# carlson-lab/redcliff-s-hypothesizing-dynamic-causal-graphs

Hardware: AMD Instinct MI355X
Metric: cMLP-factor fwd+bwd windows/sec/GPU; grid-search fits/hour on 8 GPUs (higher is better)
Workload: dtype f32; 1 GPU; REDCLIFF-S cMLP w/ state smoothing, D4IC-shaped (p=10, gen_lag=4, K=4, h=100, DGCNN F=20/2 layers/30 hidden), combined-phase batch_update, B=128; global_batch=128, parallelism=replicas1 (one independent fit per GPU, no collective), ranks=1, world_size=1

## Files before the change

redcliff-s-hypothesizing-dynamic-causal-graphs_amd/csrc/rc_common.h:

```cpp
#pragma once
#include <hip/hip_runtime.h>
#include <hip/hip_ext.h>
#include <stdint.h>
#include "redcliff_hip.h"

#define RC_BLOCK 256
#define RC_TRACE_FLOATS 32768
#define RC_LDS_LIMIT_FLOATS 16384
#define RC_LDS_MAX_FLOATS 40960
#define RC_MAX_ACTIVE 256

struct EmbOff {
  int64_t A, gcW, bnw, bnb, fc1W, fc1b, fc2W, fc2b, total;
};
struct FacOff {
  int64_t W0, b0, W1, b1, total;
};
struct WsOff {
  int64_t T;
  int64_t R;
  int64_t f1;
  int64_t w;
  int64_t a;
  int64_t y;
// ... 208 lines not shown
  put(o.w1, K * eh);
  put(o.g, K * p * d.F);
  put(o.g0, K * p);
  put(o.E, p * p * Ls);
  put(o.E0, p * p);
  put(o.dE, K * p * p * Ls);
  put(o.draw, B * K);
  o.total = x;
  if (next) *next = nr;
  return o;
}
struct CEmbCtx {
  int eh;
  float* ws; int64_t wss;
  CEmbPOff po;
  CEmbWsOff wo;
};

#define LP_FACTOR 0
#define LP_FWL1 1
#define LP_COS 2
#define LP_SMOOTH 3
#define ACC_FORECAST 0
#define ACC_FACTOR 1
#define ACC_COS 2
#define ACC_FWL1 3
#define ACC_SMOOTH 4
#define ACC_ADJ 5
#define ACC_COMBO 6
#define ACC_BATCHES 7

enum {
  RC_MG_F, RC_MG_P, RC_MG_PF, RC_MG_NF, RC_MG_K, RC_MG_M1, RC_MG_H, RC_MG_L, RC_MG_B, RC_MG_NPF, RC_MG_PH,
  RC_MG_CS, RC_MG_CSF, RC_MG_NCSF, RC_MG_CSH, RC_MG_LS, RC_MG_LSF, RC_MG_NLSF, RC_MG_LSH, RC_MG_NCH, RC_MG_ENBW,
  RC_MG_ZS, RC_MG_Q, RC_MG_NU, RC_MG_N
};

struct StepCtx {
  RedcliffDims d;
  int B, Lmax, Ls, flags, nbn;
  int Bg;
  int tA, tB;
  const float* X; int64_t xr; int64_t row0;
  const float* lab; int64_t labr;
  const double* bns; int64_t bnsr;
  float *emb, *embM, *embV; int64_t es;
  float *fac, *facM, *facV; int64_t fs;
  float *rm, *rv;
  const RedcliffReplicaHyper* hyp;
  float* ws; int64_t wss;
  double* acc;
  int* conf;
  float *gE, *gF;
  int dsN, dgN, dwN;
  int64_t dsCC, dsS, dsI;
  int fslots;
  int defer;
  EmbOff eo;
  FacOff fo;
  WsOff wo;
  int nrep, rident;
  int wait_dbg;
  uint8_t rmap[RC_MAX_ACTIVE];
  unsigned mg[RC_MG_N];
  int ewpb, enbwm, enbw;
  int fzs;
  const float* cE;
  float* cdE;
  int64_t cwss;
  const float* adt;
  int adi;
};

__host__ __device__ inline int rc_rep(const StepCtx& c, int i) { return c.rident ? i : (int)c.rmap[i]; }
inline int rc_rep_host(const StepCtx& c, int i) { return rc_rep(c, i); }

#define RC_KID_EMB_FWD 0
#define RC_KID_FAC_FWD 1
#define RC_KID_FAC_BWD 2
#define RC_KID_EMB_BWD 3
#define RC_KID_EMB_FINAL 4
#define RC_KID_FAC_MIX 5
#define RC_KID_EMB_WAIT 7
#ifdef RC_TRACE
#define RC_WG_MARK(wsbase, total, kid, end)                                                        \
  do {                                                                                            \
    if (threadIdx.x == 0 && blockIdx.y == 0 && blockIdx.z == 0 && blockIdx.x < 1024)               \
      reinterpret_cast<unsigned long long*>((wsbase) + (total) - RC_TRACE_FLOATS)[(kid) * 2048 + 2 * blockIdx.x + (end)] = \
          wall_clock64();                                                                         \
  } while (0)
#define RC_PHASE(wsbase, total, bx, i)                                                            \
  do {                                                                                            \
    if (threadIdx.x == 0 && (bx) == 0 && blockIdx.y == 0 && blockIdx.z == 0)                       \
      reinterpret_cast<unsigned long long*>((wsbase) + (total) - RC_TRACE_FLOATS)[6 * 2048 + (i)] = wall_clock64(); \
  } while (0)
#else
#define RC_WG_MARK(wsbase, total, kid, end) \
  do {                                      \
  } while (0)
#define RC_PHASE(wsbase, total, bx, i) \
  do {                                 \
  } while (0)
#endif


__device__ inline void rc_store_sc1(float* p, float v) {
  __hip_atomic_store(reinterpret_cast<unsigned*>(p), __float_as_uint(v), __ATOMIC_RELAXED, __HIP_MEMORY_SCOPE_AGENT);
}
__device__ inline float rc_load_sc1(const float* p) {
  return __uint_as_float(
      __hip_atomic_load(reinterpret_cast<unsigned*>(const_cast<float*>(p)), __ATOMIC_RELAXED, __HIP_MEMORY_SCOPE_AGENT));
}
__device__ inline void rc_store_payload(float* p, float v, bool sc1) {
  if (sc1)
    rc_store_sc1(p, v);
  else
    *p = v;
}

#define RC_PUB_DWP 0u
#define RC_PUB_ALL 16u
__device__ inline void rc_publish(unsigned* cnt, unsigned shift) {
  asm volatile("s_waitcnt vmcnt(0)" ::: "memory");
  __syncthreads();
  if (threadIdx.x == 0) __hip_atomic_fetch_add(cnt, 1u << shift, __ATOMIC_RELAXED, __HIP_MEMORY_SCOPE_AGENT);
}

#define RC_WAIT_POLLS (1u << 24)
#define RC_WAIT_POLLS_DBG (1u << 12)

__device__ inline void rc_wait_count(const unsigned* cnt, unsigned shift, unsigned target, unsigned* status, unsigned polls) {
  if (threadIdx.x == 0) {
    unsigned spins = 0;
    while (((__hip_atomic_load(const_cast<unsigned*>(cnt), __ATOMIC_RELAXED, __HIP_MEMORY_SCOPE_AGENT) >> shift) & 0xffffu) < target) {
      if (++spins >= polls) {
        __hip_atomic_fetch_add(status, 1u, __ATOMIC_RELAXED, __HIP_MEMORY_SCOPE_AGENT);
        break;
      }
      __builtin_amdgcn_s_sleep(2);
    }
  }
  __builtin_amdgcn_fence(__ATOMIC_ACQUIRE, "wavefront");
  __syncthreads();
}

__device__ inline unsigned* rc_fac_lead_cnt(const StepCtx& c, float* ws) {
  return reinterpret_cast<unsigned*>(ws + c.wo.ecnt) + c.d.p * ((c.d.H + EMB_HC - 1) / EMB_HC);
}
__device__ inline void rc_wait_leads(const StepCtx& c, float* ws, const unsigned* cnt, unsigned shift, unsigned target) {
  rc_wait_count(cnt, shift, target + (c.wait_dbg ? 1u : 0u), reinterpret_cast<unsigned*>(ws + c.wo.errw),
                c.wait_dbg ? RC_WAIT_POLLS_DBG : RC_WAIT_POLLS);
}

__device__ inline float rc_wave_sum(float v) {
#pragma unroll
  for (int o = 32; o > 0; o >>= 1) v += __shfl_xor(v, o, 64);
  return v;
}

__host__ __device__ inline int64_t rc_y_idx(const RedcliffDims& d, int slot, int kj, int b) {
  return ((int64_t)slot * d.K * d.p + kj) * d.Bmax + b;
}

__device__ inline void rc_xcd_order(int nx, int nz, int& x, int& z) {
  if ((nz & 7) != 0) return;
  const int L = x + nx * z, slot = L >> 3, q = slot / nx;
  x = slot - q * nx;
  z = (L & 7) + 8 * q;
}

__host__ __device__ inline unsigned long long rc_magic40(long long d) {
  return d > 1 ? ((1ull << 40) + (unsigned long long)d - 1) / (unsigned long long)d : 0ull;
}

struct RcDiv {
  unsigned long long m;
  int d;
  __device__ inline explicit RcDiv(int dd) : m(rc_magic40(dd)), d(dd) {}
  __device__ inline int div(int n) const {
    return d == 1 ? n : (int)(((unsigned long long)(unsigned)n * m) >> 40);
  }
  __device__ inline int mod(int n) const { return n - div(n) * d; }
};

__host__ __device__ inline unsigned rc_magic32(long long d) {
  return d > 1 ? (unsigned)(((1ull << 32) + (unsigned long long)d - 1) / (unsigned long long)d) : 0u;
}
struct RcDiv32 {
  unsigned m;
  int d;
  __device__ inline RcDiv32(int dd, unsigned mm) : m(mm), d(dd) {}
  __device__ inline explicit RcDiv32(int dd) : m(rc_magic32(dd)), d(dd) {}
  __device__ inline int div(int n) const { return d == 1 ? n : (int)__umulhi((unsigned)n, m); }
  __device__ inline int mod(int n) const { return n - div(n) * d; }
};

template <int U, int NT = RC_BLOCK, class Ld, class St>
__device__ inline void rc_stage(int N, Ld ld, St st) {
  for (int base = threadIdx.x; base < N; base += U * NT) {
    float v[U];
#pragma unroll
    for (int u = 0; u < U; ++u) {
      const int e = base + u * NT;
      v[u] = e < N ? ld(e) : 0.f;
    }
#pragma unroll
    for (int u = 0; u < U; ++u) {
      const int e = base + u * NT;
      if (e < N) st(e, v[u]);
    }
  }
}

template <int U, int NT, class Ld, class St>
struct RcSeg {
  int N;
  Ld ld;
  St st;
  float v[U];
  __device__ inline bool active(int r) const { return r * U * NT < N; }
  __device__ inline void load(int r) {
#pragma unroll
    for (int u = 0; u < U; ++u) {
      const int e = r * U * NT + u * NT + (int)threadIdx.x;
      v[u] = e < N ? ld(e) : 0.f;
    }
  }
  __device__ inline void store(int r) {
#pragma unroll
    for (int u = 0; u < U; ++u) {
      const int e = r * U * NT + u * NT + (int)threadIdx.x;
      if (e < N) st(e, v[u]);
    }
  }
};
template <int U, int NT = RC_BLOCK, class Ld, class St>
__device__ inline RcSeg<U, NT, Ld, St> rc_seg(int N, Ld ld, St st) {
  return RcSeg<U, NT, Ld, St>{N, ld, st, {}};
}
template <class... S>
__device__ inline void rc_stage_all(S&&... s) {
  for (int r = 0; (s.active(r) || ...); ++r) {
    (s.load(r), ...);
    (s.store(r), ...);
  }
}

template <int U, int NT, class Ld, class St>
struct RcSegC {
  int N;
  Ld ld;
  St st;
  float v[U];
  __device__ inline bool active(int r) const { return r * U * NT < N; }
  __device__ inline void load(int r) {
#pragma unroll
    for (int u = 0; u < U; ++u) {
      const int e0 = (r * U + u) * NT;
      if (e0 < N) v[u] = ld(min(e0 + (int)threadIdx.x, N - 1));
    }
  }
  __device__ inline void store(int r) {
#pragma unroll
    for (int u = 0; u < U; ++u) {
      const int e0 = (r * U + u) * NT, e = e0 + (int)threadIdx.x;
      if (e0 < N && e < N) st(e, v[u]);
    }
  }
};
template <int U, int NT = RC_BLOCK, class Ld, class St>
__device__ inline RcSegC<U, NT, Ld, St> rc_segc(int N, Ld ld, St st) {
  return RcSegC<U, NT, Ld, St>{N, ld, st};
}

struct RcWin {
  const float* base;
  int Tp, p, L, Q;
  unsigned mQ, mp, mL;
};
__device__ __forceinline__ RcWin rc_win(const StepCtx& c, const float* X, int b0) {
  const RedcliffDims& d = c.d;
  return RcWin{X + ((c.row0 + b0) * d.T + (c.Lmax - d.L)) * d.p, d.T * d.p, d.p, d.L, d.p * d.L,
               c.mg[RC_MG_Q], c.mg[RC_MG_P], c.mg[RC_MG_L]};
}
template <int U, int TWL, int NT>
struct RcWinSeg {
  RcWin w;
  int N, nb, q0, stride, padto;
  bool slab;
  float* tile;
  float v[U];
  __device__ __forceinline__ bool active(int r) const { return r * U * NT < N; }
  __device__ __forceinline__ void load(int r) {
    if (slab) {
      const RcDiv32 dQ(w.Q, w.mQ);
#pragma unroll
      for (int u = 0; u < U; ++u) {
        const int e0 = (r * U + u) * NT;
        if (e0 < N) {
          const int e = min(e0 + (int)threadIdx.x, N - 1), b = dQ.div(e);
          v[u] = w.base[(unsigned)(e + b * (w.Tp - w.Q))];
        }
      }
    } else {
      const RcDiv32 dL(w.L, w.mL);
#pragma unroll
      for (int u = 0; u < U; ++u) {
        const int e0 = (r * U + u) * NT;
        if (e0 < N) {
          const int e = min(e0 + (int)threadIdx.x, N - 1), b = e >> TWL, q = q0 + (e & ((1 << TWL) - 1));
          const bool in = q < w.Q;
          const int qc = in ? q : 0, ch = dL.div(qc), t = qc - ch * w.L;
          const float x = w.base[(unsigned)(b * w.Tp + t * w.p + ch)];
          v[u] = in ? x : 0.f;
        }
      }
    }
  }
  __device__ __forceinline__ void store(int r) {
    if (slab) {
      const RcDiv32 dQ(w.Q, w.mQ), dp(w.p, w.mp);
#pragma unroll
      for (int u = 0; u < U; ++u) {
        const int e0 = (r * U + u) * NT, e = e0 + (int)threadIdx.x;
        if (e0 < N && e < N) {
          const int b = dQ.div(e), s = e - b * w.Q, t = dp.div(s), ch = s - t * w.p;
          tile[b * stride + ch * w.L + t] = v[u];
        }
      }
      const int pw = padto - w.Q;
      if (r == 0 && pw > 0 && N > 0) {
        const int sh = pw <= 16 ? 4 : (pw <= 32 ? 5 : 6), col = (int)threadIdx.x & ((1 << sh) - 1);
        if (col < pw)
          for (int b = (int)threadIdx.x >> sh; b < nb; b += NT >> sh) tile[b * stride + w.Q + col] = 0.f;
      }
    } else {
#pragma unroll
      for (int u = 0; u < U; ++u) {
        const int e0 = (r * U + u) * NT, e = e0 + (int)threadIdx.x;
        if (e0 < N && e < N) tile[(e >> TWL) * stride + (e & ((1 << TWL) - 1))] = v[u];
      }
    }
  }
};
template <int U, int TWL, int NT = RC_BLOCK>
__device__ __forceinline__ RcWinSeg<U, TWL, NT> rc_win_seg(const RcWin w, bool slab, int nb, int q0, float* tile, int stride, int padto) {
  RcWinSeg<U, TWL, NT> s;
  s.w = w;
  s.N = slab ? nb * w.Q : nb << TWL;
  s.nb = nb; s.q0 = q0; s.stride = stride; s.padto = padto;
  s.slab = slab;
  s.tile = tile;
  return s;
}

__device__ inline void rc_critical_priority() { __builtin_amdgcn_s_setprio(2); }

typedef float f32x16 __attribute__((ext_vector_type(16)));
typedef float f32x4 __attribute__((ext_vector_type(4)));
__device__ inline int mf_row(int reg, int lane) { return (reg & 3) + 8 * (reg >> 2) + 4 * (lane >> 5); }

template <int NB, bool CLAMP, class LA, class LB, class PA, class PB>
__device__ __forceinline__ f32x4 rc_mfma_chain16(f32x4 acc, int n, int lg, LA la, LB lb, PA pa, PB pb) {
  for (int k0 = 0; k0 < n; k0 += 4 * NB) {
    float av[NB], bv[NB];
#pragma unroll
    for (int s = 0; s < NB; ++s) {
      const int k = k0 + 4 * s + lg, kc = CLAMP ? min(k, n - 1) : k;
      av[s] = la(kc);
      bv[s] = lb(kc);
    }
    __builtin_amdgcn_sched_barrier(0);
#pragma unroll
    for (int s = 0; s < NB; ++s) {
      const int k = k0 + 4 * s + lg;
      if (k0 + 4 * s >= n) break;
      acc = __builtin_amdgcn_mfma_f32_16x16x4f32(pa(k) ? av[s] : 0.f, pb(k) ? bv[s] : 0.f, acc, 0, 0, 0);
    }
  }
  return acc;
}
template <int NB, bool CLAMP, class LA, class LB>
__device__ __forceinline__ f32x4 rc_mfma_chain16(f32x4 acc, int n, int lg, LA la, LB lb) {
  auto in = [n](int k) { return k < n; };
  return rc_mfma_chain16<NB, CLAMP>(acc, n, lg, la, lb, in, in);
}

__device__ inline float rc_block_sum(float v, float* red) {
  v = rc_wave_sum(v);
  const int lane = threadIdx.x & 63, wv = threadIdx.x >> 6;
  __syncthreads();
  if (lane == 0) red[wv] = v;
  __syncthreads();
  float s = 0.f;
  for (int i = 0; i < (int)(blockDim.x >> 6); ++i) s += red[i];
  __syncthreads();
  return s;
// ... 181 lines not shown
```

redcliff-s-hypothesizing-dynamic-causal-graphs_amd/csrc/rc_forward.hip:

```cpp
#include <cstdlib>
#include <cstring>
#include <type_traits>

#include "rc_common.h"

namespace {

#define FK_BT 128
#define FQ_MAX 96
#define RC_EMB_TEAM_NT 512
#ifndef FF_KB
#define FF_KB 4
#endif

__device__ inline int fq_tile(const RedcliffDims& d) { return d.p * d.L <= FQ_MAX ? d.p * d.L : 32; }

template <int NBT, int NT>
__device__ __attribute__((always_inline)) void emb_fwd_body(const StepCtx& c, int bx, int SB, int w_lds, int cs, int zs, float* sm) {
  constexpr bool TEAM = NT == RC_EMB_TEAM_NT;
  constexpr int UD = NT / RC_BLOCK;
  const RedcliffDims& d = c.d;
  const int r = rc_rep(c, blockIdx.y);
  const int b0 = bx * SB;
  const int nb = min(SB, c.B - b0);
  if (nb <= 0) return;
  const int Zs = cs == (int)c.mg[RC_MG_CS] ? c.fzs : (d.p + cs - 1) / cs;
  const int zlo = zs < 0 ? 0 : zs, zhi = zs < 0 ? Zs : zs + 1;
  const int ch0 = zlo * cs, ch1 = min(d.p, zhi * cs);
  RC_WG_MARK(c.ws, c.wo.total, RC_KID_EMB_FWD, 0);
  RC_PHASE(c.ws, c.wo.total, bx, 0);
  const int p = d.p, F = d.F, H = d.H, n = d.n, M1 = d.M1, K = d.K;
  const int pF = p * F, pH = p * H, nFH = n * F * H;
  const RcDiv32 dF(F, c.mg[RC_MG_F]), dp(p, c.mg[RC_MG_P]), dpF(pF, c.mg[RC_MG_PF]), dH(H, c.mg[RC_MG_H]);
  const float* E = c.emb + r * c.es;
  float* ws = c.ws + r * c.wss;
  const float* X = c.X + r * c.xr;
  const int tid = threadIdx.x;

  float* xs = sm;
  float* Sl = xs + SB * pF;
  float* Wl = Sl + n * p * p;
  float* Tl = Wl + (w_lds ? nFH : 0);
  float* Rl = Tl + SB * n * pF;
  float* f1l = Rl + SB * pH;
  float* fc2s = f1l + SB * M1;
  float* fb1 = fc2s + K * M1;
  float* fb2 = fb1 + M1;
  float* alpha = fb2 + K;
  float* beta = alpha + F;
  float* partl = beta + F;

  if (blockIdx.x == 0) {
    unsigned* cnt = reinterpret_cast<unsigned*>(ws + c.wo.ecnt);
    for (int e = tid; e < p * rc_nchunk(d); e += NT) cnt[e] = 0u;
  }
  RC_PHASE(c.ws, c.wo.total, bx, 1);
  const bool train = c.flags & RC_BN_TRAIN;
  double st_mean = 0.0, st_var = 0.0;
  float bw = 0.f, bb = 0.f;
  if (tid < F) {
    if (train) {
      st_mean = c.bns[r * c.bnsr + tid];
      st_var = c.bns[r * c.bnsr + F + tid];
    } else {
      st_mean = c.rm[r * F + tid];
      st_var = c.rv[r * F + tid];
    }
    bw = E[c.eo.bnw + tid];
    bb = E[c.eo.bnb + tid];
  }
  const float* S = ws + c.wo.S;
  const float* gw = E + c.eo.gcW;
  rc_stage_all(
      rc_seg<2 / UD, NT>(n * p * p, [&](int e) { return S[e]; }, [&](int e, float v) { Sl[e] = v; }),
      rc_seg<20 / UD, NT>(w_lds ? nFH : 0, [&](int e) { return gw[e]; }, [&](int e, float v) { Wl[e] = v; }),
      rc_seg<4 / UD, NT>(nb * pF, [&](int e) {
        const int s = dpF.div(e), rem = e - s * pF;
        return X[(c.row0 + b0 + s) * d.T * p + (int64_t)(c.Lmax - F) * p + rem];
      }, [&](int e, float v) {
        const int s = dpF.div(e), rem = e - s * pF, f = dp.div(rem), ch = rem - f * p;
        xs[s * pF + ch * F + f] = v;
      }),
      rc_seg<4 / UD, NT>(K * M1, [&](int e) { return E[c.eo.fc2W + e]; }, [&](int e, float v) { fc2s[e] = v; }),
      rc_seg<1, NT>(M1 + K, [&](int e) { return e < M1 ? E[c.eo.fc1b + e] : E[c.eo.fc2b + e - M1]; },
                [&](int e, float v) { fb1[e] = v; }));
  RC_PHASE(c.ws, c.wo.total, bx, 2);
  if (tid < F) {
    const float mean = (float)st_mean;
    const float inv = train ? (float)(1.0 / sqrt(st_var + c.hyp[r].bn_eps))
                            : 1.0f / sqrtf((float)st_var + (float)c.hyp[r].bn_eps);
    const float a = inv * bw;
    alpha[tid] = a;
    beta[tid] = bb - mean * a;
  }
  __syncthreads();
  for (int e = tid; e < nb * pF; e += NT) {
    const int f = dF.mod(e);
    xs[e] = xs[e] * alpha[f] + beta[f];
  }
  __syncthreads();
  RC_PHASE(c.ws, c.wo.total, bx, 3);
  const int cF = (ch1 - ch0) * F, cH = (ch1 - ch0) * H;
  const int cw = ch1 - ch0;
  const int mb = cw == (int)c.mg[RC_MG_CS] ? RC_MG_CSF : (cw == (int)c.mg[RC_MG_LS] ? RC_MG_LSF : -1);
  const RcDiv32 dcF = mb >= 0 ? RcDiv32(cF, c.mg[mb]) : (cw == p ? RcDiv32(cF, c.mg[RC_MG_PF]) : RcDiv32(cF));
  const RcDiv32 dncF = mb >= 0 ? RcDiv32(n * cF, c.mg[mb + 1]) : (cw == p ? RcDiv32(n * cF, c.mg[RC_MG_NPF]) : RcDiv32(n * cF));
  const RcDiv32 dcH = mb >= 0 ? RcDiv32(cH, c.mg[mb + 2]) : (cw == p ? RcDiv32(cH, c.mg[RC_MG_PH]) : RcDiv32(cH));
  for (int e = tid; e < nb * n * cF; e += NT) {
    const int s = dncF.div(e), rs = e - s * n * cF, i = dcF.div(rs), qs = rs - i * cF;
    const int q = ch0 * F + qs, rem = i * pF + q, ch = dF.div(q), f = q - ch * F;
    float v;
    if (i == 0) {
      v = xs[s * pF + q];
    } else {
      v = 0.f;
      const float* Srow = Sl + (i * p + ch) * p;
      const float* xc = xs + s * pF + f;
      for (int cc = 0; cc < p; ++cc) v += Srow[cc] * xc[cc * F];
    }
    Tl[s * n * pF + rem] = v;
    ws[c.wo.T + (int64_t)(b0 + s) * n * pF + rem] = v;
  }
  __syncthreads();
  RC_PHASE(c.ws, c.wo.total, bx, 4);
  const float* W1 = E + c.eo.fc1W;
  const int lane = tid & 63, wv = __builtin_amdgcn_readfirstlane(tid >> 6) & 3;
  const int team = TEAM ? __builtin_amdgcn_readfirstlane(tid >> 8) : 0;
  const int fz0 = TEAM ? min(team, Zs) : zlo, fz1 = TEAM ? min(team + 1, Zs) : zhi;
  const int RW = (M1 + 3) / 4, m0 = wv * RW;
  auto qend = [&](int z) { return min(p, (z + 1) * cs) * H; };
  int qb = qend(fz0);
  auto ldw = [&](float (&w)[16], int qn) {
    const int qc = qn < qb ? qn : qb - 1;
#pragma unroll
    for (int j = 0; j < 16; ++j) w[j] = (j < RW && m0 + j < M1) ? W1[(int64_t)(m0 + j) * pH + qc] : 0.f;
  };
  float wb0[16], wb1[16], wb2[16];
  if (fz0 < fz1) {
    ldw(wb0, fz0 * cs * H + lane);
    ldw(wb1, fz0 * cs * H + lane + 64);
  }
  RC_PHASE(c.ws, c.wo.total, bx, 5);
  const float* Wsrc = w_lds ? Wl : gw;
  for (int e = tid; e < nb * cH; e += NT) {
    const int s = dcH.div(e), rem = ch0 * H + (e - s * cH), ch = dH.div(rem), hh = rem - ch * H;
    float a4[4] = {0.f, 0.f, 0.f, 0.f};
    for (int i = 0; i < n; ++i) {
      const float* trow = Tl + (s * n + i) * pF + ch * F;
      const float* wc = Wsrc + i * F * H + hh;
      int f = 0;
      for (; f + 3 < F; f += 4) {
#pragma unroll
        for (int u = 0; u < 4; ++u) a4[u] += trow[f + u] * wc[(f + u) * H];
      }
      for (; f < F; ++f) a4[0] += trow[f] * wc[f * H];
    }
    const float v = fmaxf((a4[0] + a4[1]) + (a4[2] + a4[3]), 0.f);
    Rl[s * pH + rem] = v;
    ws[c.wo.R + (int64_t)(b0 + s) * pH + rem] = v;
  }
  __syncthreads();
  RC_PHASE(c.ws, c.wo.total, bx, 6);
  const int jrow = (lane >> 2) & 15, mrow = m0 + jrow;
  const bool wrow = (lane & 3) == 0 && jrow < RW && mrow < M1;
  auto fc1 = [&](auto nbc) {
    constexpr int NB = decltype(nbc)::value;
    float tot[NB];
    for (int z = fz0; z < fz1; ++z) {
      const int qa = z * cs * H;
      qb = qend(z);
      if (z > fz0) {
        ldw(wb0, qa + lane);
        ldw(wb1, qa + lane + 64);
      }
      float acc[16][NB];
#pragma unroll
      for (int j = 0; j < 16; ++j)
#pragma unroll
        for (int s = 0; s < NB; ++s) acc[j][s] = 0.f;
      auto mul = [&](const float (&w)[16], int q) {
        if (q < qb) {
          float rv[NB];
#pragma unroll
          for (int s = 0; s < NB; ++s) rv[s] = s < nb ? Rl[s * pH + q] : 0.f;
#pragma unroll
          for (int j = 0; j < 16; ++j)
#pragma unroll
            for (int s = 0; s < NB; ++s) acc[j][s] += w[j] * rv[s];
        }
      };
      for (int q0 = qa; q0 < qb; q0 += 192) {
        const int q = q0 + lane;
        ldw(wb2, q + 128);
        mul(wb0, q);
        if (q0 + 64 >= qb) break;
        ldw(wb0, q + 192);
        mul(wb1, q + 64);
        if (q0 + 128 >= qb) break;
        ldw(wb1, q + 256);
        mul(wb2, q + 128);
      }
#pragma unroll
      for (int s = 0; s < NB; ++s) {
        if (s >= nb) break;
        float v[16];
#pragma unroll
        for (int j = 0; j < 16; ++j) v[j] = acc[j][s];
#pragma unroll
        for (int half = 8; half >= 1; half >>= 1) {
          const int off = half * 4;
          const bool hi = lane & off;
#pragma unroll
          for (int i = 0; i < half; ++i) {
            const float send = hi ? v[i] : v[i + half];
            const float keep = hi ? v[i + half] : v[i];
            v[i] = keep + __shfl_xor(send, off, 64);
          }
        }
        float t = v[0];
        t += __shfl_xor(t, 2, 64);
        t += __shfl_xor(t, 1, 64);
        tot[s] = z == fz0 ? t : tot[s] + t;
      }
    }
    if (TEAM) {
      if (wrow && fz0 < fz1) partl[team * M1 + mrow] = tot[0];
    } else if (zs < 0) {
#pragma unroll
      for (int s = 0; s < NB; ++s) {
        if (s >= nb) break;
        if (wrow) {
          const float val = tot[s] + fb1[mrow];
          f1l[s * M1 + mrow] = val;
          ws[c.wo.f1 + (int64_t)(b0 + s) * M1 + mrow] = val;
        }
      }
    } else if (wrow) {
      rc_store_sc1(ws + c.wo.f1p + ((int64_t)zs * d.Bmax + b0) * M1 + mrow, tot[0]);
    }
  };
  fc1(std::integral_constant<int, NBT>{});
  if (TEAM) {
    __syncthreads();
    RC_PHASE(c.ws, c.wo.total, bx, 12);
    if (tid < M1) {
      const float val = Zs > 1 ? (partl[tid] + partl[M1 + tid]) + fb1[tid] : partl[tid] + fb1[tid];
      f1l[tid] = val;
      ws[c.wo.f1 + (int64_t)b0 * M1 + tid] = val;
    }
  } else if (zs >= 0) {
    __shared__ unsigned last;
    unsigned* cnt = reinterpret_cast<unsigned*>(ws + c.wo.ecnt) + p * rc_nchunk(d) + 1 + b0;
    asm volatile("s_waitcnt vmcnt(0)" ::: "memory");
    __syncthreads();
    if (tid == 0) last = __hip_atomic_fetch_add(cnt, 1u, __ATOMIC_RELAXED, __HIP_MEMORY_SCOPE_AGENT) == (unsigned)(Zs - 1);
    __syncthreads();
    if (!last) return;
    if (tid == 0) __hip_atomic_store(cnt, 0u, __ATOMIC_RELAXED, __HIP_MEMORY_SCOPE_AGENT);
    __builtin_amdgcn_fence(__ATOMIC_ACQUIRE, "wavefront");
    if (tid < M1) {
      const float* part = ws + c.wo.f1p + (int64_t)b0 * M1 + tid;
      float sum = 0.f;
      for (int z0 = 0; z0 < Zs; z0 += 8) {
        float v[8];
#pragma unroll
        for (int u = 0; u < 8; ++u) v[u] = z0 + u < Zs ? rc_load_sc1(part + (int64_t)(z0 + u) * d.Bmax * M1) : 0.f;
#pragma unroll
        for (int u = 0; u < 8; ++u)
          if (z0 + u < Zs) sum = z0 + u == 0 ? v[0] : sum + v[u];
      }
      const float val = sum + fb1[tid];
      f1l[tid] = val;
      ws[c.wo.f1 + (int64_t)b0 * M1 + tid] = val;
    }
  }
  __syncthreads();
  RC_PHASE(c.ws, c.wo.total, bx, 7);
  for (int e = tid; e < nb * K; e += NT) {
    const int s = e / K, k = e - s * K;
    const float* w2 = fc2s + k * M1;
    float a = 0.f;
    for (int m = 0; m < M1; ++m) a += w2[m] * fmaxf(f1l[s * M1 + m], 0.f);
    ws[c.wo.w + (int64_t)(b0 + s) * K + k] = a + fb2[k];
  }
  RC_PHASE(c.ws, c.wo.total, bx, 8);
  RC_WG_MARK(c.ws, c.wo.total, RC_KID_EMB_FWD, 1);
}

size_t emb_fwd_floats(const RedcliffDims& d, int SB, int w_lds, bool team = false) {
  const size_t pF = (size_t)d.p * d.F, pH = (size_t)d.p * d.H;
  return SB * pF + (size_t)d.n * d.p * d.p + (w_lds ? (size_t)d.n * d.F * d.H : 0) + SB * d.n * pF + SB * pH +
         (size_t)SB * d.M1 + (size_t)d.K * d.M1 + d.M1 + d.K + 2 * d.F + (team ? 2 * d.M1 : 0);
}

template <int NT, bool MF>
__device__ __attribute__((always_inline)) void fac_fwd_body(const StepCtx& c, int bx, float* sm) {
  constexpr int UD = NT / RC_BLOCK, NI = FK_BT * FAC_UC / NT;
  const RedcliffDims& d = c.d;
  RC_WG_MARK(c.ws, c.wo.total, RC_KID_FAC_FWD, 0);
  const int nU = rc_nuchunk(d);
  const int r = rc_rep(c, blockIdx.y), kj = RcDiv32(nU, c.mg[RC_MG_NU]).div(bx), uc = bx - kj * nU;
  const int p = d.p, h = d.h, K = d.K;
  const int Q = p * d.L, QT = fq_tile(d), QP = QT + 1;
  const bool slab = Q <= FQ_MAX;
  const int u0 = uc * FAC_UC;
  const float* P = c.fac + r * c.fs;
  const float* W0 = P + c.fo.W0 + (int64_t)kj * h * Q;
  const float* b0 = P + c.fo.b0 + (int64_t)kj * h;
  const float* W1 = P + c.fo.W1 + (int64_t)kj * h;
  const float b1 = uc == 0 ? P[c.fo.b1 + kj] : 0.f;
  float* ws = c.ws + r * c.wss;
  const float* X = c.X + r * c.xr;
  const int tid = threadIdx.x, tb = tid >> 4, tu = tid & 15;
  const int u = u0 + tu;
  const RcDiv32 dQ(Q, c.mg[RC_MG_Q]);
  float* Xs = sm;
  float* Ws = Xs + FK_BT * QP;
  const int nrow = min(FAC_UC, h - u0);
  const float* W0c = W0 + u0 * Q;
  const float bu = u < h ? b0[u] : 0.f, w1 = u < h ? W1[u] : 0.f;
  const bool mf = MF && slab;
  const int lane = tid & 63, fwv = __builtin_amdgcn_readfirstlane(tid >> 6), l15 = lane & 15, lg = lane >> 4;
  float bu4[4], w14[4];
#pragma unroll
  for (int reg = 0; reg < 4; ++reg) {
    const int uu = u0 + 4 * lg + reg;
    bu4[reg] = mf && uu < h ? b0[uu] : 0.f;
    w14[reg] = mf && uu < h ? W1[uu] : 0.f;
  }

  for (int bc = 0; bc < c.B; bc += FK_BT) {
    float acc[NI];
#pragma unroll
    for (int i = 0; i < NI; ++i) acc[i] = 0.f;
    for (int q0 = 0; q0 < Q; q0 += QT) {
      if (q0 > 0 || bc > 0) __syncthreads();
      rc_stage_all(
          rc_win_seg<24 / UD, 5, NT>(rc_win(c, X, bc), slab, min(FK_BT, c.B - bc), q0, Xs, QP, Q),
          rc_segc<4 / UD, NT>(slab ? nrow * Q : 0, [&](int e) { return W0c[(unsigned)e]; }, [&](int e, float v) {
            const int uu = dQ.div(e);
            Ws[uu * QP + e - uu * Q] = v;
          }),
          rc_segc<2 / UD, NT>(slab ? 0 : FAC_UC * 32, [&](int e) {
            const int uu = e >> 5, q = q0 + (e & 31);
            const bool in = uu < nrow && q < Q;
            const float w = W0c[(unsigned)(in ? uu * Q + q : 0)];
            return in ? w : 0.f;
          }, [&](int e, float v) { Ws[(e >> 5) * QP + (e & 31)] = v; }));
      if (slab)
        for (int e = nrow * QP + tid; e < FAC_UC * QP; e += NT) Ws[e] = 0.f;
      __syncthreads();
      if (bc == 0 && q0 == 0) RC_PHASE(c.ws, c.wo.total, bx, 64);
      if (bc == 0)
        for (int qq = tid; qq < QT && q0 + qq < Q; qq += NT) {
          float sq = 0.f;
          for (int uu = 0; uu < FAC_UC; ++uu) {
            const float w = Ws[uu * QP + qq];
            sq += w * w;
          }
          ws[c.wo.gq + ((int64_t)uc * K * p + kj) * Q + q0 + qq] = sq;
        }
      if (bc == 0 && q0 == 0) RC_PHASE(c.ws, c.wo.total, bx, 65);
      if (mf) break;
      const int qn = min(QT, Q - q0);
#pragma unroll 8
      for (int qq = 0; qq < qn; ++qq) {
        const float wv = Ws[tu * QP + qq];
#pragma unroll
        for (int i = 0; i < NI; ++i) acc[i] = fmaf(Xs[(tb + (NT / 16) * i) * QP + qq], wv, acc[i]);
      }
    }
    if (bc == 0 && tb == 0 && u < h) ws[c.wo.w1 + (int64_t)kj * h + u] = w1;
    if (mf) {
      const float* wr = Ws + l15 * QP;
      for (int bt = fwv; bt < (min(FK_BT, c.B - bc) + 15) / 16; bt += NT / 64) {
        const float* xr = Xs + (16 * bt + l15) * QP;
        const f32x4 z = rc_mfma_chain16<FF_KB, true>(
            f32x4{0.f, 0.f, 0.f, 0.f}, Q, lg, [&](int kc) { return wr[kc]; }, [&](int kc) { return xr[kc]; });
        if (bc == 0 && bt == 0) RC_PHASE(c.ws, c.wo.total, bx, 66);
        const int b = bc + 16 * bt + l15;
        float ys[4];
#pragma unroll
        for (int reg = 0; reg < 4; ++reg) {
          const int uu = u0 + 4 * lg + reg;
          ys[reg] = 0.f;
          if (uu < h) {
            const float a = fmaxf(z[reg] + bu4[reg], 0.f);
            if (b < c.B && !rc_fac_recompute(d)) ws[c.wo.a + ((int64_t)kj * d.Bmax + b) * h + uu] = a;
            ys[reg] = w14[reg] * a;
          }
        }
#pragma unroll
        for (int reg = 0; reg < 4; ++reg) ys[reg] += __shfl_xor(ys[reg], 32, 64);
#pragma unroll
        for (int reg = 0; reg < 4; ++reg) ys[reg] += __shfl_xor(ys[reg], 16, 64);
        const float y = (ys[0] + ys[2]) + (ys[1] + ys[3]);
        if (lg == 0 && b < c.B) ws[c.wo.y + rc_y_idx(d, uc, kj, b)] = y + b1;
      }
      continue;
    }
    if (bc == 0) RC_PHASE(c.ws, c.wo.total, bx, 66);
#pragma unroll
    for (int i = 0; i < NI; ++i) {
      const int b = bc + tb + (NT / 16) * i;
      float ys = 0.f;
      if (u < h) {
        const float a = fmaxf(acc[i] + bu, 0.f);
        if (b < c.B && !rc_fac_recompute(d)) ws[c.wo.a + ((int64_t)kj * d.Bmax + b) * h + u] = a;
        ys = w1 * a;
      }
#pragma unroll
      for (int o = 8; o > 0; o >>= 1) ys += __shfl_xor(ys, o, 64);
      if (tu == 0 && b < c.B) ws[c.wo.y + rc_y_idx(d, uc, kj, b)] = ys + b1;
    }
  }
  RC_PHASE(c.ws, c.wo.total, bx, 67);
  RC_WG_MARK(c.ws, c.wo.total, RC_KID_FAC_FWD, 1);
}

size_t fac_fwd_floats(const RedcliffDims& d) {
  const int QT = d.p * d.L <= FQ_MAX ? d.p * d.L : 32;
  return (size_t)(FK_BT + FAC_UC) * (QT + 1);
}

template <int NBT, int NT, bool MF>
__global__ __launch_bounds__(NT) void k_forward(StepCtx c, int SB, int w_lds, int nemb, int cs, int split) {
  extern __shared__ float sm[];
  if (blockIdx.x == 0 && nemb > 0 && threadIdx.x == 0)
    *rc_fac_lead_cnt(c, c.ws + rc_rep(c, blockIdx.y) * c.wss) = 0u;
  if ((int)blockIdx.x < nemb) {
// ... 116 lines not shown
```

Before: 2.893 million windows/s.

## Overlap embedding fwd global loads and defer T/R stores past fc1

Folds the BN parameter loads into the LDS staging loop, with an explicit wait after each round, and issues the first fc1 weight prefetch before the BN/graph-conv stages so its latency overlaps that compute. The global stores of T and R are moved out of the compute loops into a separate pass issued after the fc1 reduction atomic, so they overlap the split-K synchronisation. The fc1 inner loop becomes branch-free with clamped indices, and prefetch of the next z-slab's weights is rotated. Risks include extra register pressure from the three live weight buffers across more code, and changed store ordering relative to later consumers of T and R.

```diff
diff --git a/redcliff-s-hypothesizing-dynamic-causal-graphs_amd/csrc/rc_common.h b/redcliff-s-hypothesizing-dynamic-causal-graphs_amd/csrc/rc_common.h
--- a/redcliff-s-hypothesizing-dynamic-causal-graphs_amd/csrc/rc_common.h
+++ b/redcliff-s-hypothesizing-dynamic-causal-graphs_amd/csrc/rc_common.h
@@ -384,6 +384,14 @@
                 c.wait_dbg ? RC_WAIT_POLLS_DBG : RC_WAIT_POLLS);
 }
 
+template <class T>
+__device__ inline T rc_keep(T v) {
+  asm volatile("" : "+v"(v) : : "memory");
+  return v;
+}
+
+__device__ inline void rc_wait_loads() { __builtin_amdgcn_s_waitcnt(0x0F70); }
+
 __device__ inline float rc_wave_sum(float v) {
 #pragma unroll
   for (int o = 32; o > 0; o >>= 1) v += __shfl_xor(v, o, 64);
@@ -475,6 +483,29 @@
   for (int r = 0; (s.active(r) || ...); ++r) {
     (s.load(r), ...);
     (s.store(r), ...);
+  }
+}
+
+template <class Ld>
+struct RcSegOnce {
+  Ld ld;
+  __device__ inline bool active(int r) const { return r == 0; }
+  __device__ inline void load(int r) {
+    if (r == 0) ld();
+  }
+  __device__ inline void store(int) {}
+};
+template <class Ld>
+__device__ inline RcSegOnce<Ld> rc_seg_once(Ld ld) {
+  return RcSegOnce<Ld>{ld};
+}
+
+template <class... S>
+__device__ inline void rc_stage_all_closed(S&&... s) {
+  for (int r = 0; (s.active(r) || ...); ++r) {
+    (s.load(r), ...);
+    (s.store(r), ...);
+    rc_wait_loads();
   }
 }
 
diff --git a/redcliff-s-hypothesizing-dynamic-causal-graphs_amd/csrc/rc_forward.hip b/redcliff-s-hypothesizing-dynamic-causal-graphs_amd/csrc/rc_forward.hip
--- a/redcliff-s-hypothesizing-dynamic-causal-graphs_amd/csrc/rc_forward.hip
+++ b/redcliff-s-hypothesizing-dynamic-causal-graphs_amd/csrc/rc_forward.hip
@@ -57,21 +57,26 @@
   RC_PHASE(c.ws, c.wo.total, bx, 1);
   const bool train = c.flags & RC_BN_TRAIN;
   double st_mean = 0.0, st_var = 0.0;
+  float rn_mean = 0.f, rn_var = 0.f;
   float bw = 0.f, bb = 0.f;
-  if (tid < F) {
-    if (train) {
-      st_mean = c.bns[r * c.bnsr + tid];
-      st_var = c.bns[r * c.bnsr + F + tid];
-    } else {
-      st_mean = c.rm[r * F + tid];
-      st_var = c.rv[r * F + tid];
-    }
-    bw = E[c.eo.bnw + tid];
-    bb = E[c.eo.bnb + tid];
-  }
+  double bn_eps = 0.0;
   const float* S = ws + c.wo.S;
   const float* gw = E + c.eo.gcW;
-  rc_stage_all(
+  rc_stage_all_closed(
+      rc_seg_once([&]() {
+        if (tid < F) {
+          if (train) {
+            st_mean = c.bns[r * c.bnsr + tid];
+            st_var = c.bns[r * c.bnsr + F + tid];
+          } else {
+            rn_mean = c.rm[r * F + tid];
+            rn_var = c.rv[r * F + tid];
+          }
+          bw = E[c.eo.bnw + tid];
+          bb = E[c.eo.bnb + tid];
+          bn_eps = c.hyp[r].bn_eps;
+        }
+      }),
       rc_seg<2 / UD, NT>(n * p * p, [&](int e) { return S[e]; }, [&](int e, float v) { Sl[e] = v; }),
       rc_seg<20 / UD, NT>(w_lds ? nFH : 0, [&](int e) { return gw[e]; }, [&](int e, float v) { Wl[e] = v; }),
       rc_seg<4 / UD, NT>(nb * pF, [&](int e) {
@@ -85,10 +90,30 @@
       rc_seg<1, NT>(M1 + K, [&](int e) { return e < M1 ? E[c.eo.fc1b + e] : E[c.eo.fc2b + e - M1]; },
                 [&](int e, float v) { fb1[e] = v; }));
   RC_PHASE(c.ws, c.wo.total, bx, 2);
+  const float* W1 = E + c.eo.fc1W;
+  const int lane = tid & 63, wv = __builtin_amdgcn_readfirstlane(tid >> 6) & 3;
+  const int team = TEAM ? __builtin_amdgcn_readfirstlane(tid >> 8) : 0;
+  const int fz0 = TEAM ? min(team, Zs) : zlo, fz1 = TEAM ? min(team + 1, Zs) : zhi;
+  const int RW = (M1 + 3) / 4, m0 = wv * RW;
+  auto qend = [&](int z) { return min(p, (z + 1) * cs) * H; };
+  int qb = qend(fz0);
+  auto ldw = [&](float (&w)[16], int qn) {
+    const int qc = qn < qb ? qn : qb - 1;
+#pragma unroll
+    for (int j = 0; j < 16; ++j) w[j] = W1[(int64_t)min(m0 + j, M1 - 1) * pH + qc];
+  };
+  float wb0[16], wb1[16], wb2[16];
+  rc_wait_loads();
+  auto ldw3 = [&](int qa) {
+    ldw(wb0, qa + lane);
+    if (qa + 64 < qb) ldw(wb1, qa + lane + 64);
+    if (qa + 128 < qb) ldw(wb2, qa + lane + 128);
+  };
+  if (fz0 < fz1) ldw3(fz0 * cs * H);
   if (tid < F) {
-    const float mean = (float)st_mean;
-    const float inv = train ? (float)(1.0 / sqrt(st_var + c.hyp[r].bn_eps))
-                            : 1.0f / sqrtf((float)st_var + (float)c.hyp[r].bn_eps);
+    const float mean = train ? (float)rc_keep(st_mean) : rc_keep(rn_mean);
+    const double eps = rc_keep(bn_eps);
+    const float inv = train ? (float)(1.0 / sqrt(rc_keep(st_var) + eps)) : 1.0f / sqrtf(rc_keep(rn_var) + (float)eps);
     const float a = inv * bw;
     alpha[tid] = a;
     beta[tid] = bb - mean * a;
@@ -119,47 +144,41 @@
       for (int cc = 0; cc < p; ++cc) v += Srow[cc] * xc[cc * F];
     }
     Tl[s * n * pF + rem] = v;
-    ws[c.wo.T + (int64_t)(b0 + s) * n * pF + rem] = v;
   }
   __syncthreads();
   RC_PHASE(c.ws, c.wo.total, bx, 4);
-  const float* W1 = E + c.eo.fc1W;
-  const int lane = tid & 63, wv = __builtin_amdgcn_readfirstlane(tid >> 6) & 3;
-  const int team = TEAM ? __builtin_amdgcn_readfirstlane(tid >> 8) : 0;
-  const int fz0 = TEAM ? min(team, Zs) : zlo, fz1 = TEAM ? min(team + 1, Zs) : zhi;
-  const int RW = (M1 + 3) / 4, m0 = wv * RW;
-  auto qend = [&](int z) { return min(p, (z + 1) * cs) * H; };
-  int qb = qend(fz0);
-  auto ldw = [&](float (&w)[16], int qn) {
-    const int qc = qn < qb ? qn : qb - 1;
-#pragma unroll
-    for (int j = 0; j < 16; ++j) w[j] = (j < RW && m0 + j < M1) ? W1[(int64_t)(m0 + j) * pH + qc] : 0.f;
+  auto gconv = [&](auto* Wsrc) {
+    for (int e = tid; e < nb * cH; e += NT) {
+      const int s = dcH.div(e), rem = ch0 * H + (e - s * cH), ch = dH.div(rem), hh = rem - ch * H;
+      float a4[4] = {0.f, 0.f, 0.f, 0.f};
+      for (int i = 0; i < n; ++i) {
+        const float* trow = Tl + (s * n + i) * pF + ch * F;
+        auto* wc = Wsrc + i * F * H + hh;
+        int f = 0;
+        for (; f + 3 < F; f += 4) {
+#pragma unroll
+          for (int u = 0; u < 4; ++u) a4[u] += trow[f + u] * wc[(f + u) * H];
+        }
+        for (; f < F; ++f) a4[0] += trow[f] * wc[f * H];
+      }
+      Rl[s * pH + rem] = fmaxf((a4[0] + a4[1]) + (a4[2] + a4[3]), 0.f);
+    }
   };
-  float wb0[16], wb1[16], wb2[16];
-  if (fz0 < fz1) {
-    ldw(wb0, fz0 * cs * H + lane);
-    ldw(wb1, fz0 * cs * H + lane + 64);
-  }
-  RC_PHASE(c.ws, c.wo.total, bx, 5);
-  const float* Wsrc = w_lds ? Wl : gw;
-  for (int e = tid; e < nb * cH; e += NT) {
-    const int s = dcH.div(e), rem = ch0 * H + (e - s * cH), ch = dH.div(rem), hh = rem - ch * H;
-    float a4[4] = {0.f, 0.f, 0.f, 0.f};
-    for (int i = 0; i < n; ++i) {
-      const float* trow = Tl + (s * n + i) * pF + ch * F;
-      const float* wc = Wsrc + i * F * H + hh;
-      int f = 0;
-      for (; f + 3 < F; f += 4) {
-#pragma unroll
-        for (int u = 0; u < 4; ++u) a4[u] += trow[f + u] * wc[(f + u) * H];
-      }
-      for (; f < F; ++f) a4[0] += trow[f] * wc[f * H];
-    }
-    const float v = fmaxf((a4[0] + a4[1]) + (a4[2] + a4[3]), 0.f);
-    Rl[s * pH + rem] = v;
-    ws[c.wo.R + (int64_t)(b0 + s) * pH + rem] = v;
-  }
+  if (w_lds)
+    gconv(Wl);
+  else
+    gconv(gw);
   __syncthreads();
+  auto store_TR = [&]() {
+    for (int e = tid; e < nb * n * cF; e += NT) {
+      const int s = dncF.div(e), rs = e - s * n * cF, i = dcF.div(rs), rem = i * pF + ch0 * F + (rs - i * cF);
+      ws[c.wo.T + (int64_t)(b0 + s) * n * pF + rem] = Tl[s * n * pF + rem];
+    }
+    for (int e = tid; e < nb * cH; e += NT) {
+      const int s = dcH.div(e), rem = ch0 * H + (e - s * cH);
+      ws[c.wo.R + (int64_t)(b0 + s) * pH + rem] = Rl[s * pH + rem];
+    }
+  };
   RC_PHASE(c.ws, c.wo.total, bx, 6);
   const int jrow = (lane >> 2) & 15, mrow = m0 + jrow;
   const bool wrow = (lane & 3) == 0 && jrow < RW && mrow < M1;
@@ -169,36 +188,40 @@
     for (int z = fz0; z < fz1; ++z) {
       const int qa = z * cs * H;
       qb = qend(z);
-      if (z > fz0) {
-        ldw(wb0, qa + lane);
-        ldw(wb1, qa + lane + 64);
-      }
       float acc[16][NB];
 #pragma unroll
       for (int j = 0; j < 16; ++j)
 #pragma unroll
         for (int s = 0; s < NB; ++s) acc[j][s] = 0.f;
       auto mul = [&](const float (&w)[16], int q) {
-        if (q < qb) {
-          float rv[NB];
-#pragma unroll
-          for (int s = 0; s < NB; ++s) rv[s] = s < nb ? Rl[s * pH + q] : 0.f;
-#pragma unroll
-          for (int j = 0; j < 16; ++j)
-#pragma unroll
-            for (int s = 0; s < NB; ++s) acc[j][s] += w[j] * rv[s];
-        }
+        const int qc = q < qb ? q : qb - 1;
+        float rv[NB];
+#pragma unroll
+        for (int s = 0; s < NB; ++s) {
+          const float x = Rl[(s < nb ? s : 0) * pH + qc];
+          rv[s] = s < nb && q < qb ? x : 0.f;
+        }
+#pragma unroll
+        for (int j = 0; j < 16; ++j)
+#pragma unroll
+          for (int s = 0; s < NB; ++s) acc[j][s] += w[j] * rv[s];
       };
       for (int q0 = qa; q0 < qb; q0 += 192) {
         const int q = q0 + lane;
-        ldw(wb2, q + 128);
         mul(wb0, q);
-        if (q0 + 64 >= qb) break;
-        ldw(wb0, q + 192);
-        mul(wb1, q + 64);
-        if (q0 + 128 >= qb) break;
-        ldw(wb1, q + 256);
-        mul(wb2, q + 128);
+        if (q0 + 192 < qb) ldw(wb0, q + 192);
+        if (q0 + 64 < qb) {
+          mul(wb1, q + 64);
+          if (q0 + 256 < qb) ldw(wb1, q + 256);
+        }
+        if (q0 + 128 < qb) {
+          mul(wb2, q + 128);
+          if (q0 + 320 < qb) ldw(wb2, q + 320);
+        }
+      }
+      if (!TEAM && z + 1 < fz1) {
+        qb = qend(z + 1);
+        ldw3((z + 1) * cs * H);
       }
 #pragma unroll
       for (int s = 0; s < NB; ++s) {
@@ -253,7 +276,10 @@
     unsigned* cnt = reinterpret_cast<unsigned*>(ws + c.wo.ecnt) + p * rc_nchunk(d) + 1 + b0;
     asm volatile("s_waitcnt vmcnt(0)" ::: "memory");
     __syncthreads();
-    if (tid == 0) last = __hip_atomic_fetch_add(cnt, 1u, __ATOMIC_RELAXED, __HIP_MEMORY_SCOPE_AGENT) == (unsigned)(Zs - 1);
+    unsigned seen = 0u;
+    if (tid == 0) seen = __hip_atomic_fetch_add(cnt, 1u, __ATOMIC_RELAXED, __HIP_MEMORY_SCOPE_AGENT);
+    store_TR();
+    if (tid == 0) last = seen == (unsigned)(Zs - 1);
     __syncthreads();
     if (!last) return;
     if (tid == 0) __hip_atomic_store(cnt, 0u, __ATOMIC_RELAXED, __HIP_MEMORY_SCOPE_AGENT);
@@ -276,6 +302,7 @@
   }
   __syncthreads();
   RC_PHASE(c.ws, c.wo.total, bx, 7);
+  if (zs < 0) store_TR();
   for (int e = tid; e < nb * K; e += NT) {
     const int s = e / K, k = e - s * K;
     const float* w2 = fc2s + k * M1;
```

New measurement: 3.041 million windows/s, median of 6. 1.05x the previous value.
